# yflyl613/Tiny-NewsRec

Measured on AMD Instinct MI355X. Metric: training impressions/sec, higher is better.
Workload: dtype fp16; 1 GPU; Tiny-NewsRec 4-layer student (train [2, 3]) + 4-teacher KD (title-emb MSE + soft-CE), fwd+bwd+AMSGrad; batch_per_gpu=32, global_batch=32, user_log_length=50, candidates=5, num_words_title=30, news_dim=256, n_news=51282, parallelism=dp1

## Files before the change

include/tnr_hip.h:

```cpp
#ifndef TNR_HIP_H
#define TNR_HIP_H
#include <stdint.h>

#ifdef __cplusplus
extern "C" {
#endif

#define TNR_OK 0
#define TNR_EINVAL (-1)
#define TNR_EUNSUPPORTED (-2)
#define TNR_ELAUNCH (-3)

#define TNR_BF16 0
#define TNR_F16 1
#define TNR_F32 2

#define TNR_EPI_BIAS 1
#define TNR_EPI_GELU 2
#define TNR_EPI_TANH 4
#define TNR_EPI_RES 8
#define TNR_EPI_MULDGELU 16
#define TNR_EPI_OUTF32 32
#define TNR_EPI_AUXOUT 64
#define TNR_EPI_COLSUM 128
// ... 175 lines not shown
                         int64_t M, int64_t N, int64_t K, const float* bias, const void* res, int64_t ldres,
                         void* aux, int64_t ldaux, int flags, float* colsum_part, const tnr_dropout_t* drop,
                         const tnr_dropout_t* drop_tail, int64_t split_row, void* stream);
int tnr_ln_bwd_do_split(const void* dy, const void* x, const float* stats, const float* gamma, void* dx,
                        float* dgamma, float* dbeta, float* dxsum, float* part, int64_t M, int H, void* dxm,
                        const tnr_dropout_t* drop, const tnr_dropout_t* drop_tail, int64_t split_row, void* stream);
int tnr_attn_l32_fwd_do(const void* qkv, const float* mask_add, const float* rel, void* ctx, int64_t n_seq, int L, int A,
                        const tnr_dropout_t* drop, void* stream);
int tnr_attn_l32_bwd_do(const void* qkv, const float* mask_add, const float* rel, const void* dctx, void* dqkv,
                        float* bias_part, int64_t n_seq, int L, int A, const tnr_dropout_t* drop, void* stream);
int tnr_attn_long_fwd_do(const void* qkv, const float* mask_add, const float* rel, void* ctx, float* lse, int64_t n_seq,
                         int L, int A, const tnr_dropout_t* drop, void* stream);
int tnr_attn_long_bwd_do(const void* qkv, const float* mask_add, const float* rel, const void* ctx, const void* dctx,
                         const float* lse, float* delta, void* dqkv, int64_t n_seq, int L, int A,
                         const tnr_dropout_t* drop, void* stream);
int tnr_dropout_mask(const tnr_dropout_t* drop, int64_t rows, int64_t cols, float* out, void* stream);
int tnr_dropout_mask_probs(const tnr_dropout_t* drop, int64_t pairs, int L, int by_columns, float* out, void* stream);
int tnr_dropout_mask_split(const tnr_dropout_t* drop, const tnr_dropout_t* drop_tail, int64_t split_row, int64_t rows, int64_t cols,
                           float* out, void* stream);


int tnr_amsgrad_step(float* p, const float* g, float* m, float* v, float* vmax, int64_t n, int step,
                     float lr, float beta1, float beta2, float eps, float grad_scale, void* stream);

int tnr_grad_nonfinite(const float* g, int64_t n, unsigned* guard, unsigned stamp, void* stream);
int tnr_grad_nonfinite_scan(const float* g, int64_t n, unsigned* guard, unsigned stamp, void* stream);
int tnr_grad_nonfinite_commit(unsigned* guard, unsigned stamp, void* stream);
int tnr_amsgrad_step_guarded(float* p, const float* g, float* m, float* v, float* vmax, int64_t n, int step,
                             float lr, float beta1, float beta2, float eps, float grad_scale, const unsigned* guard,
                             unsigned stamp, unsigned known_skips, void* stream);

int tnr_refresh_shadows(const int64_t* desc, int n_desc, int64_t total_tiles, const int64_t* tile_start,
                        void* stream);

int tnr_cast_f32_to_bf16(const float* src, void* dst, int64_t n, void* stream);
int tnr_cast_bf16_to_f32(const void* src, float* dst, int64_t n, void* stream);

int tnr_embed_ln_fwd_f16(const int64_t* tok, int64_t n_seq, int L, int H, const float* word, const float* pos,
                     const float* type0, const float* gamma, const float* beta, float eps,
                     void* out, float* mask_add, void* stream);
int tnr_embed_ln_fwd_indexed_f16(const int32_t* news_combined, const int32_t* nidx, int64_t n_seq, int L, int H,
                             const float* word, const float* pos, const float* type0, const float* gamma,
                             const float* beta, float eps, void* out, float* mask_add, void* stream);
int tnr_gemm_nt_f16(const void* A, int64_t lda, const void* B, int64_t ldb, void* C, int64_t ldc,
                int64_t M, int64_t N, int64_t K, const float* bias, const void* res, int64_t ldres,
                void* aux, int64_t ldaux, int flags, void* stream);
int tnr_gemm_nt_ex_f16(const void* A, int64_t lda, const void* B, int64_t ldb, void* C, int64_t ldc,
                   int64_t M, int64_t N, int64_t K, const float* bias, const void* res, int64_t ldres,
                   void* aux, int64_t ldaux, int flags, float* colsum_part, void* stream);
int64_t tnr_gemm_colsum_rows_f16(int64_t M);
int tnr_gemm_nt_route_f16(int64_t M, int64_t N, int64_t K, int flags);
int tnr_gemm_tn_wgrad_f16(const void* dY, int64_t lddy, const void* X, int64_t ldx, float* dW, int64_t lddw,
                      int64_t M, int64_t N, int64_t K, float* ws, int splits, int accumulate, void* stream);
int tnr_gemm_tn_wgrad_ex_f16(const void* dY, int64_t lddy, const void* X, int64_t ldx, float* dW, int64_t lddw,
                         int64_t M, int64_t N, int64_t K, float* ws, int splits, int accumulate, float out_scale,
                         void* stream);
int64_t tnr_gemm_tn_ws_elems_f16(int64_t N, int64_t K, int splits);
int tnr_gemm_tn_wgrad_group_f16(const tnr_wgrad_problem_t* problems, int n, void* stream);
int tnr_ln_fwd_f16(const void* x, const float* gamma, const float* beta, float eps, void* y, float* stats,
               int64_t M, int H, void* stream);
int tnr_ln_bwd_f16(const void* dy, const void* x, const float* stats, const float* gamma, void* dx,
               float* dgamma, float* dbeta, float* dxsum, float* part, int64_t M, int H, void* stream);
int tnr_pool_fwd_f16(const void* y, float* nv, int64_t n_seq, int L, int H, int mean, void* stream);
int tnr_pool_bwd_f16(const float* dnv, void* dy, int64_t n_seq, int L, int H, int mean, void* stream);
int tnr_attn_long_fwd_f16(const void* qkv, const float* mask_add, const float* rel, void* ctx, float* lse,
                          int64_t n_seq, int L, int A, void* stream);
int tnr_attn_long_bwd_f16(const void* qkv, const float* mask_add, const float* rel, const void* ctx, const void* dctx,
                          const float* lse, float* delta, void* dqkv, int64_t n_seq, int L, int A, void* stream);
int tnr_attn_l32_fwd_f16(const void* qkv, const float* mask_add, const float* rel, void* ctx,
                     int64_t n_seq, int L, int A, void* stream);
int tnr_attn_l32_bwd_f16(const void* qkv, const float* mask_add, const float* rel, const void* dctx,
                     void* dqkv, float* bias_part, int64_t n_seq, int L, int A, void* stream);
int tnr_colsum_f16(const void* X, int64_t ldx, int dtype, int64_t M, int64_t N, float* out, float* part,
               int accumulate, void* stream);
int tnr_colsum_batched_f16(const void* X, int64_t ldx, int64_t sX, int dtype, int64_t M, int64_t N, int batch,
                       float* out, float* part, int accumulate, void* stream);
int tnr_attpool_fwd_f16(const void* y, const float* e, int64_t lde, const float* w2, const float* b2, int Q,
                    float* nv, float* alpha, float* den, int64_t n_seq, int L, int H, void* stream);
int tnr_attpool_bwd_f16(const void* y, const float* e, int64_t lde, const float* w2, int Q, const float* dnv,
                    const float* alpha, const float* den, void* dy_direct, void* dpre, int64_t lddpre,
                    float* dw2_part, float* db2_part, float* db1_part, int64_t n_seq, int L, int H, void* stream);
int64_t tnr_attpool_long_ws_elems_f16(int64_t n_seq, int L, int H, int Q, int64_t lddpre);
int tnr_attpool_fwd_long_f16(const void* y, const float* e, int64_t lde, const float* w2, const float* b2, int Q,
                         float* nv, float* alpha, float* den, float* ws, int64_t n_seq, int L, int H, void* stream);
int tnr_attpool_bwd_long_f16(const void* y, const float* e, int64_t lde, const float* w2, int Q, const float* dnv,
                         const float* alpha, void* dy_direct, void* dpre, int64_t lddpre, float* dw2_part,
                         float* db2_part, float* db1_part, float* ws, int64_t n_seq, int L, int H, void* stream);
int tnr_refresh_shadows_f16(const int64_t* desc, int n_desc, int64_t total_tiles, const int64_t* tile_start,
                        void* stream);
int tnr_cast_f32_to_bf16_f16(const float* src, void* dst, int64_t n, void* stream);
int tnr_cast_bf16_to_f32_f16(const void* src, float* dst, int64_t n, void* stream);

int tnr_embed_ln_fwd_do_f16(const int64_t* tok, int64_t n_seq, int L, int H, const float* word, const float* pos,
                        const float* type0, const float* gamma, const float* beta, float eps, void* out, float* mask_add,
                        const tnr_dropout_t* drop, const int32_t* pos_ids, void* stream);
int tnr_embed_ln_fwd_indexed_do_f16(const int32_t* news_combined, const int32_t* nidx, int64_t n_seq, int L, int H,
                                const float* word, const float* pos, const float* type0, const float* gamma,
                                const float* beta, float eps, void* out, float* mask_add, const tnr_dropout_t* drop,
                                const int32_t* pos_ids, void* stream);
int tnr_gemm_nt_do_f16(const void* A, int64_t lda, const void* B, int64_t ldb, void* C, int64_t ldc,
                   int64_t M, int64_t N, int64_t K, const float* bias, const void* res, int64_t ldres,
                   void* aux, int64_t ldaux, int flags, float* colsum_part, const tnr_dropout_t* drop, void* stream);
int tnr_ln_bwd_do_f16(const void* dy, const void* x, const float* stats, const float* gamma, void* dx,
                  float* dgamma, float* dbeta, float* dxsum, float* part, int64_t M, int H, void* dxm,
                  const tnr_dropout_t* drop, void* stream);
int tnr_gemm_nt_do_split_f16(const void* A, int64_t lda, const void* B, int64_t ldb, void* C, int64_t ldc,
                             int64_t M, int64_t N, int64_t K, const float* bias, const void* res, int64_t ldres,
                             void* aux, int64_t ldaux, int flags, float* colsum_part, const tnr_dropout_t* drop,
                             const tnr_dropout_t* drop_tail, int64_t split_row, void* stream);
int tnr_ln_bwd_do_split_f16(const void* dy, const void* x, const float* stats, const float* gamma, void* dx,
                            float* dgamma, float* dbeta, float* dxsum, float* part, int64_t M, int H, void* dxm,
                            const tnr_dropout_t* drop, const tnr_dropout_t* drop_tail, int64_t split_row, void* stream);
int tnr_attn_l32_fwd_do_f16(const void* qkv, const float* mask_add, const float* rel, void* ctx, int64_t n_seq, int L, int A,
                        const tnr_dropout_t* drop, void* stream);
int tnr_attn_l32_bwd_do_f16(const void* qkv, const float* mask_add, const float* rel, const void* dctx, void* dqkv,
                        float* bias_part, int64_t n_seq, int L, int A, const tnr_dropout_t* drop, void* stream);
int tnr_attn_long_fwd_do_f16(const void* qkv, const float* mask_add, const float* rel, void* ctx, float* lse, int64_t n_seq,
                         int L, int A, const tnr_dropout_t* drop, void* stream);
int tnr_attn_long_bwd_do_f16(const void* qkv, const float* mask_add, const float* rel, const void* ctx, const void* dctx,
                         const float* lse, float* delta, void* dqkv, int64_t n_seq, int L, int A,
                         const tnr_dropout_t* drop, void* stream);

// ... 14 lines not shown
```

tiny-newsrec_amd/csrc/optim.hip:

```cpp
#include <algorithm>

#include "common.h"

namespace {

typedef __attribute__((ext_vector_type(4))) unsigned u32x4_t;

struct AdamFactors { float lr_c1[3], inv_sqrt_c2[3]; unsigned known_skips; };
template <bool AMS>
__global__ __launch_bounds__(256) void amsgrad_kernel(float* __restrict__ p, const float* __restrict__ g,
                                                      float* __restrict__ m, float* __restrict__ v,
                                                      float* __restrict__ vmax, int64_t n, AdamFactors f,
                                                      float b1, float b2, float eps, float gscale,
                                                      const unsigned* __restrict__ guard, unsigned stamp) {
    float lr_c1 = f.lr_c1[0], inv_sqrt_c2 = f.inv_sqrt_c2[0];
    if (guard) {
        if (guard[0] == stamp) return;
        const unsigned k = guard[1] - f.known_skips;
        if (k == 1) { lr_c1 = f.lr_c1[1]; inv_sqrt_c2 = f.inv_sqrt_c2[1]; }
        else if (k >= 2) { lr_c1 = f.lr_c1[2]; inv_sqrt_c2 = f.inv_sqrt_c2[2]; }
    }
    int64_t i = ((int64_t)blockIdx.x * blockDim.x + threadIdx.x) * 4;
    if (i >= n) return;
    if (i + 4 <= n) {
// ... 56 lines not shown
                                                      const int64_t* __restrict__ tile_start) {
    __shared__ float t[32][33];
    int64_t tile = blockIdx.x;
    int di = 0;
    while (di + 1 < n_desc && tile >= tile_start[di + 1]) ++di;
    const int64_t* d = desc + (int64_t)di * 8;
    const float* src = (const float*)d[0];
    const int64_t rows = d[1], cols = d[2];
    bf16* dst = (bf16*)d[3];
    const int64_t ld = d[4];
    bf16* dstT = (bf16*)d[5];
    const int64_t ldT = d[6];
    const int64_t local = tile - tile_start[di];
    const int64_t tcols = (cols + 31) / 32;
    const int64_t r0 = (local / tcols) * 32, c0 = (local % tcols) * 32;
    const int tx = threadIdx.x & 31, ty = threadIdx.x >> 5;
#pragma unroll
    for (int k = 0; k < 4; ++k) {
        int64_t r = r0 + ty + 8 * k, c = c0 + tx;
        float v = (r < rows && c < cols) ? src[r * cols + c] : 0.f;
        t[ty + 8 * k][tx] = v;
        if (dst && r < rows && c < cols) dst[r * ld + c] = (bf16)v;
    }
    __syncthreads();
    if (dstT) {
#pragma unroll
        for (int k = 0; k < 4; ++k) {
            int64_t c = c0 + ty + 8 * k, r = r0 + tx;
            if (r < rows && c < cols) dstT[c * ldT + r] = (bf16)t[tx][ty + 8 * k];
        }
    }
}

}

#ifndef TNR_BUILD_F16
extern "C" int tnr_amsgrad_step_guarded(float* p, const float* g, float* m, float* v, float* vmax, int64_t n, int step, float lr,
                                        float beta1, float beta2, float eps, float grad_scale, const unsigned* guard,
                                        unsigned stamp, unsigned known_skips, void* stream);
extern "C" int tnr_amsgrad_step(float* p, const float* g, float* m, float* v, float* vmax, int64_t n, int step, float lr,
                                float beta1, float beta2, float eps, float grad_scale, void* stream) {
    return tnr_amsgrad_step_guarded(p, g, m, v, vmax, n, step, lr, beta1, beta2, eps, grad_scale, nullptr, 0u, 0u, stream);
}

extern "C" int tnr_grad_nonfinite_scan(const float* g, int64_t n, unsigned* guard, unsigned stamp, void* stream) {
    TNR_CHECK_ARG(g && guard && n >= 1 && stamp >= 1 && ((uintptr_t)g % 16) == 0, "tnr_grad_nonfinite_scan: bad argument");
    const unsigned grid = (unsigned)std::min<int64_t>((n + 4095) / 4096, 2048);
    hipLaunchKernelGGL(grad_nonfinite_kernel, dim3(grid), dim3(256), 0, (hipStream_t)stream, g, n, guard, stamp);
    TNR_CHECK_LAUNCH("tnr_grad_nonfinite_scan");
    return TNR_OK;
}

extern "C" int tnr_grad_nonfinite_commit(unsigned* guard, unsigned stamp, void* stream) {
    TNR_CHECK_ARG(guard && stamp >= 1, "tnr_grad_nonfinite_commit: bad argument");
    hipLaunchKernelGGL(grad_nonfinite_count_kernel, dim3(1), dim3(1), 0, (hipStream_t)stream, guard, stamp);
    TNR_CHECK_LAUNCH("tnr_grad_nonfinite_commit");
    return TNR_OK;
}

extern "C" int tnr_grad_nonfinite(const float* g, int64_t n, unsigned* guard, unsigned stamp, void* stream) {
    TNR_CHECK_ARG(g && guard && n >= 1 && stamp >= 1 && ((uintptr_t)g % 16) == 0, "tnr_grad_nonfinite: bad argument");
    const unsigned grid = (unsigned)std::min<int64_t>((n + 4095) / 4096, 2048);
    hipLaunchKernelGGL(grad_nonfinite_kernel, dim3(grid), dim3(256), 0, (hipStream_t)stream, g, n, guard, stamp);
    hipLaunchKernelGGL(grad_nonfinite_count_kernel, dim3(1), dim3(1), 0, (hipStream_t)stream, guard, stamp);
    TNR_CHECK_LAUNCH("tnr_grad_nonfinite");
    return TNR_OK;
}

extern "C" int tnr_amsgrad_step_guarded(float* p, const float* g, float* m, float* v, float* vmax, int64_t n, int step, float lr,
                                        float beta1, float beta2, float eps, float grad_scale, const unsigned* guard,
                                        unsigned stamp, unsigned known_skips, void* stream) {
    TNR_CHECK_ARG(p && g && m && v && n >= 1 && step >= 1, "tnr_amsgrad_step: bad argument");
    TNR_CHECK_ARG(((uintptr_t)p % 16) == 0 && ((uintptr_t)g % 16) == 0 && ((uintptr_t)m % 16) == 0 &&
                      ((uintptr_t)v % 16) == 0 && ((uintptr_t)vmax % 16) == 0, "tnr_amsgrad_step: 16-byte alignment");
    AdamFactors f;
    for (int k = 0; k < 3; ++k) {
        const int t = step - k >= 1 ? step - k : 1;
        const double c1 = 1.0 - pow((double)beta1, t), c2 = 1.0 - pow((double)beta2, t);
        f.lr_c1[k] = (float)((double)lr / c1);
        f.inv_sqrt_c2[k] = (float)(1.0 / sqrt(c2));
    }
    f.known_skips = known_skips;
    int64_t nthr = (n + 3) / 4;
    if (vmax)
        hipLaunchKernelGGL(amsgrad_kernel<true>, dim3((unsigned)((nthr + 255) / 256)), dim3(256), 0, (hipStream_t)stream, p, g, m,
                           v, vmax, n, f, beta1, beta2, eps, grad_scale, guard, stamp);
    else
        hipLaunchKernelGGL(amsgrad_kernel<false>, dim3((unsigned)((nthr + 255) / 256)), dim3(256), 0, (hipStream_t)stream, p, g, m,
                           v, vmax, n, f, beta1, beta2, eps, grad_scale, guard, stamp);
    TNR_CHECK_LAUNCH("tnr_amsgrad_step");
    return TNR_OK;
}

#endif

extern "C" int TNR_NAME(tnr_refresh_shadows)(const int64_t* desc, int n_desc, int64_t total_tiles, const int64_t* tile_start,
                                   void* stream) {
    TNR_CHECK_ARG(desc && tile_start && n_desc >= 1 && total_tiles >= 1, "tnr_refresh_shadows: bad argument");
    hipLaunchKernelGGL(refresh_kernel, dim3((unsigned)total_tiles), dim3(256), 0, (hipStream_t)stream, desc, n_desc,
                       tile_start);
    TNR_CHECK_LAUNCH("tnr_refresh_shadows");
    return TNR_OK;
}
```

tiny-newsrec_amd/engine.py:

```python
import logging
import math
import struct

import torch

import tnr_hip as T

PFX = "student.news_encoder."
BERT = PFX + "bert_model.bert."
QPAD = 256
AP_LONG = 64


def _rup(x, m):
    return (x + m - 1) // m * m


class EngineConfig:
    def __init__(self, n_layers=4, trainable_layers=(2, 3), hidden=768, heads=12, inter=3072, news_dim=256,
                 news_query=200, user_query=200, num_teachers=4, user_log_length=50, npratio=4, num_words=30,
                 user_log_mask=False, temperature=1.0, coef=0.2, vocab=30522, max_pos=512, type_vocab=2,
                 ln_eps=1e-12, stage1=False, pooling="att", nrms_heads=0, pos_pad_id=None):
        self.stage1 = stage1
        self.pos_pad_id = pos_pad_id
# ... 114 lines not shown
        if self.table is None:
            sb = 0 if scale == 1.0 else struct.unpack("<I", struct.pack("<f", scale))[0]
            self.jobs.append((part.data_ptr(), rows, stride, n, out.data_ptr(), int(accumulate) | (sb << 32)))

    def flush(self):
        if not self.jobs:
            return
        if self.table is None:
            l1, l2 = [], []
            for part, rows, stride, n, out, acc in self.jobs:
                chunks = max(1, min(rows // 32, 16))
                per = (rows + chunks - 1) // chunks
                chunks = (rows + per - 1) // per
                for c0 in range(0, n, 64):
                    nc = min(64, n - c0)
                    if chunks > 1:
                        for ch in range(chunks):
                            r0 = ch * per
                            src = part + 4 * (r0 * stride + c0)
                            l1.append((src, min(per, rows - r0), stride, nc, src, 0))
                        l2.append((part + 4 * c0, chunks, per * stride, nc, out + 4 * c0, acc))
                    else:
                        l2.append((part + 4 * c0, rows, stride, nc, out + 4 * c0, acc))
            mk = lambda rows_: (torch.tensor(rows_, dtype=torch.int64, device=self.dev), len(rows_)) if rows_ else None
            self.table = (mk(l1), mk(l2))
        for t in self.table:
            if t is not None:
                T.call("tnr_reduce_multi", t[0], t[1])


LOSS_SCALE = 1024.0


class LossScaler:

    def __init__(self, dev, enabled, growth_interval=2000, max_mult=64.0, min_mult=2.0 ** -20):
        self.enabled = bool(enabled) and torch.device(dev).type == "cuda"
        self.mult, self.stamp, self.clean, self.skipped, self.run_of_skips = 1.0, 0, 0, 0, 0
        self.growth_interval, self.max_mult, self.min_mult = growth_interval, max_mult, min_mult
        self.guard = torch.zeros(4, dtype=torch.int32, device=dev) if self.enabled else None
        self.pending = []
        self._ring = torch.zeros(8, dtype=torch.int32).pin_memory() if self.enabled else None

    def poll(self, eng, lag=2):
        while self.pending and self.pending[0][0] <= self.stamp - lag + 1:
            stamp, host, ev, used = self.pending.pop(0)
            ev.synchronize()
            if int(host[0]) == stamp:
                self.skipped += 1
                self.clean = 0
                self.run_of_skips += 1
                self.mult = max(min(self.mult, used * 0.5), self.min_mult)
                eng.step_count = max(eng.step_count - 1, 0)
                if self.run_of_skips == 16:
                    logging.warning("16 optimiser steps in a row skipped for inf / nan gradients although the loss scale went down "
                                    "to %g: the fp16 FORWARD overflows (or the data holds inf / nan) - use --dtype bf16", eng.gscale)
            else:
                self.run_of_skips = 0
                self.clean += 1
                if self.clean >= self.growth_interval and self.mult < self.max_mult:
                    self.mult, self.clean = self.mult * 2.0, 0

    def record(self, used):
        host = self._ring[self.stamp % 8: self.stamp % 8 + 1]
        host.copy_(self.guard[:1], non_blocking=True)
        ev = torch.cuda.Event()
        ev.record()
        self.pending.append((self.stamp, host, ev, used))

    def drain(self, eng):
        self.poll(eng, lag=0)

    def reset(self, eng):
        self.drain(eng)
        self.mult, self.clean, self.run_of_skips = 1.0, 0, 0


class Engine:
    def __init__(self, cfg, device="cuda:0", max_batch=32, dtype="fp16", share=None, extra_rows=0, extra_seqs=0):
        T.lib()
        assert dtype in ("bf16", "fp16")
        self.f16 = dtype == "fp16"
        self.dtype = dtype
        self.tdt = torch.float16 if self.f16 else torch.bfloat16
        self._gbase = LOSS_SCALE if self.f16 else 1.0
        self.cfg, self.dev = cfg, torch.device(device)
        self.scaler = share.scaler if share is not None else LossScaler(self.dev, self.f16)
        self.step_count = 0
        self._n_alloc = 0
        if share is None:
            self._build_params()
            self._build_shadows()
        else:
            for k in ("shapes", "slot", "n_train", "n_frozen", "flat", "flat_g", "adam_m", "adam_v", "adam_vmax", "params",
                      "grads", "lo", "sh", "sh_a1", "sh_a1T", "b_a1", "desc_all", "desc_train"):
                setattr(self, k, getattr(share, k))
        self.max_batch = max_batch
        self.extra_rows, self.extra_seqs = int(extra_rows), int(extra_seqs)
        self.drop = None
        self.drop_calls = 0
        self._alloc_workspace(max_batch)
        self.comm = None

    @property
    def gscale(self):
        return self._gbase * self.scaler.mult

    @property
    def ginv(self):
        return 1.0 / self.gscale

    def _groups(self):
        cfg = self.cfg
        T_ = cfg.T
        tstack = lambda suffix: ["teachers.%d.%s" % (i, suffix) for i in range(T_)]
        groups = []
        if T_ and cfg.nrms_heads and not cfg.stage1:
            groups.append((["teachers.%d.%s" % (i, n) for i in range(T_) for n in NRMS_W], None))
            groups.append((["teachers.%d.%s" % (i, n) for i in range(T_) for n in NRMS_B], None))
        if T_ and not cfg.stage1:
            for suffix in ("attn.att_fc1.weight", "attn.att_fc1.bias", "attn.att_fc2.weight", "pad_doc", "attn.att_fc2.bias"):
                groups.append((tstack(suffix), None))
        for k in ("word_embeddings.weight", "position_embeddings.weight", "token_type_embeddings.weight",
                  "LayerNorm.weight", "LayerNorm.bias"):
            groups.append(([BERT + "embeddings." + k], None))
        for l in range(cfg.n_layers):
            n = layer_param_order(l)
            groups.append((n[0:3], None))
# ... 113 lines not shown
        cfg, dev, bf = self.cfg, self.dev, self.tdt
        H, I = cfg.H, cfg.I
        lo = min(cfg.trainable_layers) if cfg.trainable_layers else cfg.n_layers
        self.lo = lo
        self.sh = []
        for l in range(cfg.n_layers):
            d = dict(qkv=torch.zeros((3 * H, H), device=dev, dtype=bf), o=torch.zeros((H, H), device=dev, dtype=bf),
                     w1=torch.zeros((I, H), device=dev, dtype=bf), w2=torch.zeros((H, I), device=dev, dtype=bf))
            if l >= lo:
                d.update(qkvT=torch.zeros((H, 3 * H), device=dev, dtype=bf), oT=torch.zeros((H, H), device=dev, dtype=bf),
                         w1T=torch.zeros((H, I), device=dev, dtype=bf), w2T=torch.zeros((I, H), device=dev, dtype=bf))
            self.sh.append(d)
        self.sh_a1 = torch.zeros((QPAD, H), device=dev, dtype=bf)
        self.sh_a1T = torch.zeros((H, QPAD), device=dev, dtype=bf)
        self.b_a1 = self._view(PFX + "attn.att_fc1.bias", QPAD, (QPAD,)) if cfg.pooling == "att" else None

        def table(layers, with_heads):
            rows = []
            for l in layers:
                d, names = self.sh[l], layer_param_order(l)
                for i in range(3):
                    rows.append((self.p(names[i]), H, H, d["qkv"][i * H:], H, d["qkvT"][:, i * H:] if "qkvT" in d else None, 3 * H))
                rows.append((self.p(names[6]), H, H, d["o"], H, d.get("oT"), H))
                rows.append((self.p(names[10]), I, H, d["w1"], H, d.get("w1T"), I))
                rows.append((self.p(names[12]), H, I, d["w2"], I, d.get("w2T"), H))
            if with_heads and cfg.pooling == "att":
                rows.append((self.p(PFX + "attn.att_fc1.weight"), cfg.Qn, H, self.sh_a1, H, self.sh_a1T, QPAD))
            desc, start, tot = [], [0], 0
            for src, r, c, dst, ld, dstT, ldT in rows:
                desc.append([src.data_ptr(), r, c, dst.data_ptr(), ld, dstT.data_ptr() if dstT is not None else 0, ldT, 0])
                tot += ((r + 31) // 32) * ((c + 31) // 32)
                start.append(tot)
            return (torch.tensor(desc, dtype=torch.int64, device=dev), len(desc), tot,
                    torch.tensor(start, dtype=torch.int64, device=dev))

        self.desc_all = table(range(cfg.n_layers), True)
        self.desc_train = table(cfg.trainable_layers, True)

    def refresh_shadows(self, all_layers=False):
        d = self.desc_all if all_layers else self.desc_train
        self._c("tnr_refresh_shadows", d[0], d[1], d[2], d[3])
        if all_layers:
            self.fcache = None
            self.refresh_rel()

    def refresh_rel(self):
        T.call("tnr_relpos_table", self.p(BERT + "rel_pos_bias.weight"), self.cfg.A, self.cfg.L, self.rel)
        self._rel_stale = False

    def _alloc_workspace(self, B):
        cfg, dev, bf = self.cfg, self.dev, self.tdt
        H, I, D, L = cfg.H, cfg.I, cfg.D, cfg.L
        N = B * (cfg.U + cfg.C)
        Mp = _rup(N * L + self.extra_rows, 128)
        self.B_alloc, self.N_alloc, self.Mp = B, N, Mp
        Nx = N + self.extra_seqs
        if self.f16:
            k = 0
            while (32 << k) < B and k < 5:
                k += 1
            self._gbase = LOSS_SCALE * (1 << k)
        z = lambda *s, dt=bf: torch.zeros(s, device=dev, dtype=dt)
        f = lambda *s: torch.zeros(s, device=dev, dtype=torch.float32)
        Lr = _rup(L, 32)
        self.Lr = Lr
        self.tok = torch.zeros((N, 2 * L), device=dev, dtype=torch.int64)
        self.nidx_buf = torch.zeros(N, device=dev, dtype=torch.int32)
        self.mask_add = f(N, Lr)
        self.rel = f(cfg.A, Lr, Lr)
        self.lse = f(N, cfg.A, Lr) if L > 32 else None
# ... 638 lines not shown
    def grad(self, name):
        return self.grads[name]

    def bucket_ranges(self):
        out = [(self.off(PFX + ("attn.att_fc1.weight" if self.cfg.pooling == "att" else "dense.weight")), self.n_train)]
        for l in sorted(self.cfg.trainable_layers, reverse=True):
            names = layer_param_order(l)
            a0, f0 = self.off(names[0]), self.off(names[10])
            e = self.off(names[-1]) + self.slot[names[-1]][2]
            out.append((f0, _rup(e, 64)))
            out.append((a0, f0))
        return out

    def step(self, lr, grad_scale=1.0, beta1=0.9, beta2=0.999, eps=1e-8, lr_bert=None, amsgrad=True, lr_news_head=None, sync=None):
        sc = self.scaler
        guard, stamp = None, 0
        if sc.enabled:
            used = sc.mult
            sc.poll(self)
            sc.stamp += 1
            guard, stamp = sc.guard, sc.stamp
        self.step_count += 1
        head0 = self.off(PFX + ("attn.att_fc1.weight" if self.cfg.pooling == "att" else "dense.weight"))
        e = self.off(PFX + "dense.bias") + self.slot[PFX + "dense.bias"][2]
        rest0 = min(_rup(e, 64), self.n_train)
        lb = lr if lr_bert is None else lr_bert
        lh = lr if lr_news_head is None else lr_news_head
        ranges = []
        for lo_, hi_, rate in ((0, head0, lb), (head0, rest0, lh), (rest0, self.n_train, lr)):
            if ranges and ranges[-1][2] == rate and ranges[-1][1] == lo_:
                ranges[-1] = (ranges[-1][0], hi_, rate)
            elif hi_ > lo_:
                ranges.append((lo_, hi_, rate))
        def launch(lo_, hi_, rate):
            if hi_ > lo_:
                args = (self.flat[True][lo_:hi_], self.flat_g[lo_:hi_], self.adam_m[lo_:hi_], self.adam_v[lo_:hi_],
                        self.adam_vmax[lo_:hi_] if amsgrad else None, hi_ - lo_, self.step_count, rate, beta1, beta2, eps, grad_scale)
                if guard is None:
                    T.call("tnr_amsgrad_step", *args)
                else:
                    T.call("tnr_amsgrad_step_guarded", *args, guard, stamp, sc.skipped)

        if guard is not None:
            if sync is not None and sync.pending:
                for b, (s_, e_) in enumerate(sync.ranges):
                    sync.wait_bucket(b)
                    T.call("tnr_grad_nonfinite_scan", self.flat_g[s_:e_], e_ - s_, guard, stamp)
                T.call("tnr_grad_nonfinite_commit", guard, stamp)
            else:
                if sync is not None:
                    sync.wait()
                T.call("tnr_grad_nonfinite", self.flat_g, self.n_train, guard, stamp)
            for lo_, hi_, rate in ranges:
                launch(lo_, hi_, rate)
            sc.record(used)
        elif sync is not None and sync.pending:
            done = []
            for b, (s_, e_) in enumerate(sync.ranges):
                sync.wait_bucket(b)
                for lo_, hi_, rate in ranges:
                    launch(max(lo_, s_), min(hi_, e_), rate)
                done.append((s_, e_))
            pos = 0
            for s_, e_ in sorted(done) + [(self.n_train, self.n_train)]:
                for lo_, hi_, rate in ranges:
                    launch(max(lo_, pos), min(hi_, s_), rate)
                pos = max(pos, e_)
        else:
            if sync is not None:
                sync.wait()
            for lo_, hi_, rate in ranges:
                launch(lo_, hi_, rate)
        self.refresh_shadows(all_layers=False)
```

tiny-newsrec_amd/tnr_hip.py:

```python
import ctypes
import os

import torch

_HERE = os.path.dirname(os.path.abspath(__file__))
LIB_PATH = os.path.join(_HERE, "csrc", "libtnr_hip.so")

BF16, F16, F32 = 0, 1, 2
ROUTE_128, ROUTE_256x128, ROUTE_256, ROUTE_224 = 128, 2128, 256, 224
EPI_BIAS, EPI_GELU, EPI_TANH, EPI_RES, EPI_MULDGELU, EPI_OUTF32, EPI_AUXOUT, EPI_COLSUM = 1, 2, 4, 8, 16, 32, 64, 128

_c = ctypes
_P, _I, _L, _F = _c.c_void_p, _c.c_int, _c.c_int64, _c.c_float

DROP_EMB, DROP_PROB, DROP_ATTN_OUT, DROP_FFN_OUT = 0, 1, 2, 3


class Dropout(_c.Structure):
    _fields_ = [("seed", _c.c_uint64), ("site", _c.c_uint32), ("call", _c.c_uint32), ("p", _c.c_double)]

    @classmethod
    def site_of(cls, p, seed, kind, layer, call):
        if p is None or p <= 0.0:
            return None
# ... 93 lines not shown
    "tnr_attpool_fwd": [_P, _P, _L, _P, _P, _I, _P, _P, _P, _L, _I, _I, _P],
    "tnr_attpool_bwd": [_P, _P, _L, _P, _I, _P, _P, _P, _P, _P, _L, _P, _P, _P, _L, _I, _I, _P],
    "tnr_attpool_fwd_long": [_P, _P, _L, _P, _P, _I, _P, _P, _P, _P, _L, _I, _I, _P],
    "tnr_attpool_bwd_long": [_P, _P, _L, _P, _I, _P, _P, _P, _P, _L, _P, _P, _P, _P, _L, _I, _I, _P],
    "tnr_sgemm": [_P, _L, _L, _L, _P, _P, _L, _L, _L, _P, _L, _L, _P, _L, _L, _L, _L, _I, _F, _F, _I, _P, _P],
    "tnr_sgemm_group": [_c.POINTER(SgemmProblem), _I, _P],
    "tnr_gemm_tn_wgrad_group": [_c.POINTER(WgradProblem), _I, _P],
    "tnr_concat_i32": [_P, _L, _P, _L, _P, _P],
    "tnr_gather_rows": [_P, _L, _P, _L, _I, _I, _P, _L, _L, _P],
    "tnr_segment_sum_rows": [_P, _P, _P, _L, _I, _P, _P],
    "tnr_user_score_fwd": [_P, _L, _P, _P, _P, _P, _P, _P, _P, _P, _I, _P, _P, _P, _L, _P, _P, _P, _P, _I, _I, _I, _I, _I, _I, _P],
    "tnr_user_bwd_pre": [_P, _P, _P, _P, _P, _I, _P, _P, _P, _P, _P, _P, _I, _I, _I, _I, _P],
    "tnr_user_bwd_post": [_P, _P, _P, _P, _P, _I, _P, _P, _I, _I, _I, _I, _P],
    "tnr_user_bwd_part_stride": [_I, _I],
    "tnr_user_blend_fwd": [_P, _L, _P, _P, _P, _I, _P, _I, _I, _I, _I, _P],
    "tnr_user_blend_bwd": [_P, _P, _P, _I, _P, _P, _L, _I, _I, _I, _P],
    "tnr_nrms_attn_fwd": [_P, _P, _I, _P, _L, _I, _I, _I, _I, _P],
    "tnr_nrms_attn_bwd": [_P, _P, _I, _P, _P, _I, _I, _I, _P],
    "tnr_score_bwd": [_P, _P, _P, _P, _P, _P, _I, _I, _I, _P],
    "tnr_kd_score_loss": [_P, _P, _P, _F, _F, _P, _P, _P, _I, _I, _I, _P],
    "tnr_kd_embed_loss": [_P, _P, _P, _P, _P, _P, _P, _I, _I, _I, _I, _I, _P],
    "tnr_reduce_rows": [_P, _L, _L, _L, _P, _I, _P],
    "tnr_reduce_multi": [_P, _I, _P],
    "tnr_dropout_mask": [_D, _L, _L, _P, _P],
    "tnr_dropout_mask_probs": [_D, _L, _I, _I, _P, _P],
    "tnr_dropout_mask_split": [_D, _D, _L, _L, _L, _P, _P],
    "tnr_scale_inplace": [_P, _L, _F, _P],
    "tnr_amsgrad_step": [_P, _P, _P, _P, _P, _L, _I, _F, _F, _F, _F, _F, _P],
    "tnr_amsgrad_step_guarded": [_P, _P, _P, _P, _P, _L, _I, _F, _F, _F, _F, _F, _P, _c.c_uint, _c.c_uint, _P],
    "tnr_grad_nonfinite": [_P, _L, _P, _c.c_uint, _P],
    "tnr_grad_nonfinite_scan": [_P, _L, _P, _c.c_uint, _P],
    "tnr_grad_nonfinite_commit": [_P, _c.c_uint, _P],
    "tnr_refresh_shadows": [_P, _I, _L, _P, _P],
    "tnr_cast_f32_to_bf16": [_P, _P, _L, _P],
    "tnr_cast_bf16_to_f32": [_P, _P, _L, _P],
}
TYPED = ["tnr_embed_ln_fwd", "tnr_embed_ln_fwd_indexed", "tnr_gemm_nt", "tnr_gemm_nt_ex", "tnr_gemm_colsum_rows", "tnr_gemm_nt_route",
         "tnr_gemm_tn_wgrad", "tnr_gemm_tn_wgrad_ex", "tnr_gemm_tn_wgrad_group", "tnr_gemm_tn_ws_elems", "tnr_ln_fwd", "tnr_ln_bwd", "tnr_attn_l32_fwd", "tnr_attn_l32_bwd", "tnr_attn_long_fwd", "tnr_attn_long_bwd",
         "tnr_colsum", "tnr_colsum_batched", "tnr_attpool_fwd", "tnr_attpool_bwd", "tnr_attpool_fwd_long", "tnr_attpool_bwd_long", "tnr_attpool_long_ws_elems", "tnr_refresh_shadows",
         "tnr_cast_f32_to_bf16", "tnr_cast_bf16_to_f32", "tnr_pool_fwd", "tnr_pool_bwd"]
for _n in ("tnr_embed_ln_fwd", "tnr_embed_ln_fwd_indexed", "tnr_attn_l32_fwd", "tnr_attn_l32_bwd", "tnr_attn_long_fwd", "tnr_attn_long_bwd"):
    _SIG[_n + "_do"] = _SIG[_n][:-1] + [_D] + ([_P] if "embed" in _n else []) + [_P]
    TYPED.append(_n + "_do")
_SIG["tnr_gemm_nt_do"] = _SIG["tnr_gemm_nt_ex"][:-1] + [_D, _P]
_SIG["tnr_ln_bwd_do"] = _SIG["tnr_ln_bwd"][:-1] + [_P, _D, _P]
_SIG["tnr_gemm_nt_do_split"] = _SIG["tnr_gemm_nt_do"][:-1] + [_D, _L, _P]
_SIG["tnr_ln_bwd_do_split"] = _SIG["tnr_ln_bwd_do"][:-1] + [_D, _L, _P]
TYPED += ["tnr_gemm_nt_do", "tnr_ln_bwd_do", "tnr_gemm_nt_do_split", "tnr_ln_bwd_do_split"]
for _n in TYPED:
    _SIG[_n + "_f16"] = _SIG[_n]
_RET = {"tnr_attpool_long_ws_elems": _L, "tnr_attpool_long_ws_elems_f16": _L, "tnr_gemm_tn_ws_elems": _L, "tnr_gemm_tn_ws_elems_f16": _L, "tnr_gemm_colsum_rows_f16": _L, "tnr_gemm_colsum_rows": _L, "tnr_ln_bwd_part_elems": _L, "tnr_ln_bwd_blocks": _L, "tnr_colsum_part_elems": _L,
        "tnr_user_bwd_part_stride": _L}
EXPORTS = sorted(_SIG) + ["tnr_last_error"]

_lib = None


class TnrError(RuntimeError):
    pass


def lib():
    global _lib
    if _lib is None:
        if not os.path.exists(LIB_PATH):
            raise TnrError("libtnr_hip.so not built: run `make -C tiny-newsrec_amd/csrc` (or __graft_entry__.build())")
        L = ctypes.CDLL(LIB_PATH)
        for name, args in _SIG.items():
            fn = getattr(L, name)
            fn.argtypes = args
            fn.restype = _RET.get(name, _I)
        L.tnr_last_error.restype = ctypes.c_char_p
# ... 75 lines not shown
```

Before: 4242 impressions/s.

## Fuse AMSGrad step with bf16 shadow weight refresh in one kernel

Adds a kernel that runs the AMSGrad update per 64x64 tile of each trainable weight matrix and writes the bf16 shadow copy and its transpose straight from registers through shared memory. Parameter ranges outside any matrix are updated as flat 4096-element chunks. This removes the separate shadow-refresh pass that re-read the updated fp32 parameters, and saves a launch. The cost is a descriptor table built and cached per optimizer range, plus more complex tail handling.

```diff
diff --git a/include/tnr_hip.h b/include/tnr_hip.h
--- a/include/tnr_hip.h
+++ b/include/tnr_hip.h
@@ -231,6 +231,11 @@
 
 int tnr_refresh_shadows(const int64_t* desc, int n_desc, int64_t total_tiles, const int64_t* tile_start,
                         void* stream);
+
+int tnr_amsgrad_step_refresh(float* p, const float* g, float* m, float* v, float* vmax, int64_t n, int step,
+                             float lr, float beta1, float beta2, float eps, float grad_scale, const unsigned* guard,
+                             unsigned stamp, unsigned known_skips, const int64_t* desc, int n_desc, int64_t total_units,
+                             const int64_t* unit_start, void* stream);
 
 int tnr_cast_f32_to_bf16(const float* src, void* dst, int64_t n, void* stream);
 int tnr_cast_bf16_to_f32(const void* src, float* dst, int64_t n, void* stream);
@@ -287,6 +292,10 @@
                          float* db2_part, float* db1_part, float* ws, int64_t n_seq, int L, int H, void* stream);
 int tnr_refresh_shadows_f16(const int64_t* desc, int n_desc, int64_t total_tiles, const int64_t* tile_start,
                         void* stream);
+int tnr_amsgrad_step_refresh_f16(float* p, const float* g, float* m, float* v, float* vmax, int64_t n, int step,
+                             float lr, float beta1, float beta2, float eps, float grad_scale, const unsigned* guard,
+                             unsigned stamp, unsigned known_skips, const int64_t* desc, int n_desc, int64_t total_units,
+                             const int64_t* unit_start, void* stream);
 int tnr_cast_f32_to_bf16_f16(const float* src, void* dst, int64_t n, void* stream);
 int tnr_cast_bf16_to_f32_f16(const void* src, float* dst, int64_t n, void* stream);
 
diff --git a/tiny-newsrec_amd/csrc/optim.hip b/tiny-newsrec_amd/csrc/optim.hip
--- a/tiny-newsrec_amd/csrc/optim.hip
+++ b/tiny-newsrec_amd/csrc/optim.hip
@@ -112,6 +112,198 @@
     }
 }
 
+AdamFactors adam_factors(int step, float lr, float beta1, float beta2, unsigned known_skips) {
+    AdamFactors f;
+    for (int k = 0; k < 3; ++k) {
+        const int t = step - k >= 1 ? step - k : 1;
+        const double c1 = 1.0 - pow((double)beta1, t), c2 = 1.0 - pow((double)beta2, t);
+        f.lr_c1[k] = (float)((double)lr / c1);
+        f.inv_sqrt_c2[k] = (float)(1.0 / sqrt(c2));
+    }
+    f.known_skips = known_skips;
+    return f;
+}
+
+struct AdamArgs { float lr_c1, inv_sqrt_c2, b1, b2, eps, gscale; };
+template <bool AMS>
+__device__ __forceinline__ void adam_update4(f32x4 graw, f32x4& mv, f32x4& vv, f32x4& vm, f32x4& pv, const AdamArgs& a) {
+    const float b1 = a.b1, b2 = a.b2, eps = a.eps, lr_c1 = a.lr_c1, inv_sqrt_c2 = a.inv_sqrt_c2;
+    f32x4 gv = graw * a.gscale;
+    mv = mv * b1 + (1.f - b1) * gv;
+    vv = vv * b2 + (1.f - b2) * gv * gv;
+    if (!AMS) vm = vv;
+#pragma unroll
+    for (int r = 0; r < 4; ++r) {
+        if (AMS) vm[r] = fmaxf(vm[r], vv[r]);
+        pv[r] -= lr_c1 * (mv[r] / (sqrtf(vm[r]) * inv_sqrt_c2 + eps));
+    }
+}
+template <bool AMS>
+__device__ __forceinline__ float adam_update1(float* p, const float* g, float* m, float* v, float* vmax, int64_t i, const AdamArgs& a) {
+    const float b1 = a.b1, b2 = a.b2, eps = a.eps, lr_c1 = a.lr_c1, inv_sqrt_c2 = a.inv_sqrt_c2;
+    float gv = g[i] * a.gscale;
+    float mv = m[i] * b1 + (1.f - b1) * gv;
+    float vv = v[i] * b2 + (1.f - b2) * gv * gv;
+    float vm = AMS ? fmaxf(vmax[i], vv) : vv;
+    m[i] = mv; v[i] = vv;
+    if (AMS) vmax[i] = vm;
+    p[i] -= lr_c1 * (mv / (sqrtf(vm) * inv_sqrt_c2 + eps));
+    return p[i];
+}
+
+template <bool AMS>
+__device__ __forceinline__ void adam_update_some(float* p, const float* g, float* m, float* v, float* vmax, int64_t i, int cnt,
+                                                 int64_t tail, const AdamArgs& a, float out[4]) {
+    f32x4 G = {0.f, 0.f, 0.f, 0.f}, M = G, V = G, X = G, P = G;
+#pragma unroll
+    for (int j = 0; j < 4; ++j)
+        if (j < cnt && i + j < tail) {
+            G[j] = g[i + j]; M[j] = m[i + j]; V[j] = v[i + j]; P[j] = p[i + j];
+            if (AMS) X[j] = vmax[i + j];
+        }
+    adam_update4<AMS>(G, M, V, X, P, a);
+#pragma unroll
+    for (int j = 0; j < 4; ++j)
+        if (j < cnt) {
+            if (i + j < tail) {
+                m[i + j] = M[j]; v[i + j] = V[j]; p[i + j] = P[j];
+                if (AMS) vmax[i + j] = X[j];
+                out[j] = P[j];
+            } else {
+                out[j] = adam_update1<AMS>(p, g, m, v, vmax, i + j, a);
+            }
+        }
+}
+
+constexpr int FT = 64;
+constexpr int FCHUNK = 4096;
+template <bool AMS>
+__global__ __launch_bounds__(256) void amsgrad_refresh_kernel(float* __restrict__ p, const float* __restrict__ g,
+                                                              float* __restrict__ m, float* __restrict__ v,
+                                                              float* __restrict__ vmax, int64_t n, AdamFactors f,
+                                                              float b1, float b2, float eps, float gscale,
+                                                              const unsigned* __restrict__ guard, unsigned stamp,
+                                                              const int64_t* __restrict__ desc, int n_desc,
+                                                              const int64_t* __restrict__ unit_start) {
+    __shared__ __attribute__((aligned(16))) bf16 tT[FT][FT + 4];
+    AdamArgs a = {f.lr_c1[0], f.inv_sqrt_c2[0], b1, b2, eps, gscale};
+    if (guard) {
+        if (guard[0] == stamp) return;
+        const unsigned k = guard[1] - f.known_skips;
+        if (k == 1) { a.lr_c1 = f.lr_c1[1]; a.inv_sqrt_c2 = f.inv_sqrt_c2[1]; }
+        else if (k >= 2) { a.lr_c1 = f.lr_c1[2]; a.inv_sqrt_c2 = f.inv_sqrt_c2[2]; }
+    }
+    const int64_t unit = blockIdx.x;
+    int di = 0, hi = n_desc - 1;
+    while (di < hi) {
+        const int mid = (di + hi + 1) >> 1;
+        if (unit_start[mid] <= unit) di = mid; else hi = mid - 1;
+    }
+    const int64_t* d = desc + (int64_t)di * 8;
+    const int64_t rows = d[1], cols = d[2];
+    const int64_t off = (const float*)d[0] - p;
+    if (rows < 1 || cols < 1 || off < 0 || off + rows * cols > n) return;
+    bf16* dst = (bf16*)d[3];
+    const int64_t ld = d[4];
+    bf16* dstT = (bf16*)d[5];
+    const int64_t ldT = d[6];
+    const int64_t local = unit - unit_start[di];
+    const int tid = threadIdx.x;
+    p += off; g += off; m += off; v += off;
+    if (AMS) vmax += off;
+    const int64_t tail = (n & ~(int64_t)3) - off;
+    const bool vec_in = (off & 3) == 0;
+
+    if (!dst && !dstT) {
+        const int64_t len = rows * cols, e0 = local * FCHUNK;
+        f32x4 G[4], M[4], V[4], X[4], P[4];
+        bool full[4];
+#pragma unroll
+        for (int u = 0; u < 4; ++u) {
+            const int64_t i = e0 + tid * 4 + u * 1024;
+            full[u] = vec_in && i + 4 <= len;
+            if (full[u]) {
+                G[u] = *(const f32x4*)(g + i); M[u] = *(const f32x4*)(m + i); V[u] = *(const f32x4*)(v + i);
+                if (AMS) X[u] = *(const f32x4*)(vmax + i);
+                P[u] = *(const f32x4*)(p + i);
+            }
+        }
+#pragma unroll
+        for (int u = 0; u < 4; ++u) {
+            const int64_t i = e0 + tid * 4 + u * 1024;
+            if (full[u]) {
+                adam_update4<AMS>(G[u], M[u], V[u], X[u], P[u], a);
+                *(f32x4*)(m + i) = M[u]; *(f32x4*)(v + i) = V[u];
+                if (AMS) *(f32x4*)(vmax + i) = X[u];
+                *(f32x4*)(p + i) = P[u];
+            } else {
+                float out[4];
+                if (i < len) adam_update_some<AMS>(p, g, m, v, vmax, i, (int)(len - i < 4 ? len - i : 4), tail, a, out);
+            }
+        }
+        return;
+    }
+
+    const int64_t tcols = (cols + FT - 1) / FT;
+    const int64_t r0 = (local / tcols) * FT, c0 = (local % tcols) * FT;
+    if (r0 >= rows) return;
+    const int lx = tid & 15, ly = tid >> 4;
+    const bool vec_row = vec_in && (cols & 3) == 0;
+    const bool vec_dst = dst && (ld & 3) == 0 && ((uintptr_t)dst & 7) == 0;
+    const int64_t c = c0 + 4 * lx;
+    f32x4 G[4], M[4], V[4], X[4], P[4];
+    bool full[4];
+#pragma unroll
+    for (int k = 0; k < 4; ++k) {
+        const int64_t r = r0 + ly + 16 * k, i = r * cols + c;
+        full[k] = vec_row && r < rows && c + 4 <= cols;
+        if (full[k]) {
+            G[k] = *(const f32x4*)(g + i); M[k] = *(const f32x4*)(m + i); V[k] = *(const f32x4*)(v + i);
+            if (AMS) X[k] = *(const f32x4*)(vmax + i);
+            P[k] = *(const f32x4*)(p + i);
+        }
+    }
+#pragma unroll
+    for (int k = 0; k < 4; ++k) {
+        const int rl = ly + 16 * k;
+        const int64_t r = r0 + rl, i = r * cols + c;
+        if (full[k]) {
+            adam_update4<AMS>(G[k], M[k], V[k], X[k], P[k], a);
+            *(f32x4*)(m + i) = M[k]; *(f32x4*)(v + i) = V[k];
+            if (AMS) *(f32x4*)(vmax + i) = X[k];
+            *(f32x4*)(p + i) = P[k];
+            bf16x4 h;
+#pragma unroll
+            for (int j = 0; j < 4; ++j) { h[j] = (bf16)P[k][j]; tT[4 * lx + j][rl] = h[j]; }
+            if (vec_dst) *(bf16x4*)(dst + r * ld + c) = h;
+            else if (dst)
+                for (int j = 0; j < 4; ++j) dst[r * ld + c + j] = h[j];
+        } else if (r < rows) {
+            float out[4];
+            const int cnt = (int)(cols - c < 4 ? cols - c : 4);
+            if (cnt > 0) adam_update_some<AMS>(p, g, m, v, vmax, i, cnt, tail, a, out);
+            for (int j = 0; j < cnt; ++j) {
+                const bf16 h = (bf16)out[j];
+                tT[4 * lx + j][rl] = h;
+                if (dst) dst[r * ld + c + j] = h;
+            }
+        }
+    }
+    if (!dstT) return;
+    __syncthreads();
+    const bool vec_T = (ldT & 3) == 0 && ((uintptr_t)dstT & 7) == 0;
+    const int64_t r = r0 + 4 * lx;
+#pragma unroll
+    for (int k = 0; k < 4; ++k) {
+        const int cl = ly + 16 * k;
+        const int64_t cc = c0 + cl;
+        if (cc >= cols) continue;
+        if (vec_T && r + 4 <= rows) *(bf16x4*)(dstT + cc * ldT + r) = *(const bf16x4*)&tT[cl][4 * lx];
+        else
+            for (int j = 0; j < 4 && r + j < rows; ++j) dstT[cc * ldT + r + j] = tT[cl][4 * lx + j];
+    }
+}
+
 }
 
 #ifndef TNR_BUILD_F16
@@ -153,14 +345,7 @@
     TNR_CHECK_ARG(p && g && m && v && n >= 1 && step >= 1, "tnr_amsgrad_step: bad argument");
     TNR_CHECK_ARG(((uintptr_t)p % 16) == 0 && ((uintptr_t)g % 16) == 0 && ((uintptr_t)m % 16) == 0 &&
                       ((uintptr_t)v % 16) == 0 && ((uintptr_t)vmax % 16) == 0, "tnr_amsgrad_step: 16-byte alignment");
-    AdamFactors f;
-    for (int k = 0; k < 3; ++k) {
-        const int t = step - k >= 1 ? step - k : 1;
-        const double c1 = 1.0 - pow((double)beta1, t), c2 = 1.0 - pow((double)beta2, t);
-        f.lr_c1[k] = (float)((double)lr / c1);
-        f.inv_sqrt_c2[k] = (float)(1.0 / sqrt(c2));
-    }
-    f.known_skips = known_skips;
+    const AdamFactors f = adam_factors(step, lr, beta1, beta2, known_skips);
     int64_t nthr = (n + 3) / 4;
     if (vmax)
         hipLaunchKernelGGL(amsgrad_kernel<true>, dim3((unsigned)((nthr + 255) / 256)), dim3(256), 0, (hipStream_t)stream, p, g, m,
@@ -182,3 +367,24 @@
     TNR_CHECK_LAUNCH("tnr_refresh_shadows");
     return TNR_OK;
 }
+
+extern "C" int TNR_NAME(tnr_amsgrad_step_refresh)(float* p, const float* g, float* m, float* v, float* vmax, int64_t n, int step,
+                                                  float lr, float beta1, float beta2, float eps, float grad_scale,
+                                                  const unsigned* guard, unsigned stamp, unsigned known_skips,
+                                                  const int64_t* desc, int n_desc, int64_t total_units, const int64_t* unit_start,
+                                                  void* stream) {
+    TNR_CHECK_ARG(p && g && m && v && n >= 1 && step >= 1, "tnr_amsgrad_step_refresh: bad argument");
+    TNR_CHECK_ARG(((uintptr_t)p % 16) == 0 && ((uintptr_t)g % 16) == 0 && ((uintptr_t)m % 16) == 0 &&
+                      ((uintptr_t)v % 16) == 0 && ((uintptr_t)vmax % 16) == 0, "tnr_amsgrad_step_refresh: 16-byte alignment");
+    TNR_CHECK_ARG(desc && unit_start && n_desc >= 1 && total_units >= 1 && total_units <= 0x7FFFFFFF,
+                  "tnr_amsgrad_step_refresh: bad descriptor table");
+    const AdamFactors f = adam_factors(step, lr, beta1, beta2, known_skips);
+    if (vmax)
+        hipLaunchKernelGGL(amsgrad_refresh_kernel<true>, dim3((unsigned)total_units), dim3(256), 0, (hipStream_t)stream, p, g, m, v,
+                           vmax, n, f, beta1, beta2, eps, grad_scale, guard, stamp, desc, n_desc, unit_start);
+    else
+        hipLaunchKernelGGL(amsgrad_refresh_kernel<false>, dim3((unsigned)total_units), dim3(256), 0, (hipStream_t)stream, p, g, m, v,
+                           vmax, n, f, beta1, beta2, eps, grad_scale, guard, stamp, desc, n_desc, unit_start);
+    TNR_CHECK_LAUNCH("tnr_amsgrad_step_refresh");
+    return TNR_OK;
+}
diff --git a/tiny-newsrec_amd/engine.py b/tiny-newsrec_amd/engine.py
--- a/tiny-newsrec_amd/engine.py
+++ b/tiny-newsrec_amd/engine.py
@@ -170,6 +170,25 @@
 LOSS_SCALE = 1024.0
 
 
+FUSED_TILE, FUSED_CHUNK = 64, 4096
+
+
+def fused_rows(mats, lo, hi):
+    out, pos = [], lo
+    flat = lambda a, b: out.append((a, 1, b - a, None, -(-(b - a) // FUSED_CHUNK)))
+    for i, (o, r, c) in sorted(enumerate(mats), key=lambda t: t[1][0]):
+        if not lo <= o < hi:
+            continue
+        assert o >= pos and o + r * c <= hi, "weight matrix at %d (%d x %d) overlaps its neighbour or leaves [%d, %d)" % (o, r, c, lo, hi)
+        if o > pos:
+            flat(pos, o)
+        out.append((o, r, c, i, -(-r // FUSED_TILE) * -(-c // FUSED_TILE)))
+        pos = o + r * c
+    if hi > pos:
+        flat(pos, hi)
+    return out
+
+
 class LossScaler:
 
     def __init__(self, dev, enabled, growth_interval=2000, max_mult=64.0, min_mult=2.0 ** -20):
@@ -231,7 +250,7 @@
             self._build_shadows()
         else:
             for k in ("shapes", "slot", "n_train", "n_frozen", "flat", "flat_g", "adam_m", "adam_v", "adam_vmax", "params",
-                      "grads", "lo", "sh", "sh_a1", "sh_a1T", "b_a1", "desc_all", "desc_train"):
+                      "grads", "lo", "sh", "sh_a1", "sh_a1T", "b_a1", "desc_all", "desc_train", "rows_train", "_fused_tabs"):
                 setattr(self, k, getattr(share, k))
         self.max_batch = max_batch
         self.extra_rows, self.extra_seqs = int(extra_rows), int(extra_seqs)
@@ -411,10 +430,27 @@
                 tot += ((r + 31) // 32) * ((c + 31) // 32)
                 start.append(tot)
             return (torch.tensor(desc, dtype=torch.int64, device=dev), len(desc), tot,
-                    torch.tensor(start, dtype=torch.int64, device=dev))
-
-        self.desc_all = table(range(cfg.n_layers), True)
-        self.desc_train = table(cfg.trainable_layers, True)
+                    torch.tensor(start, dtype=torch.int64, device=dev), rows)
+
+        self.desc_all = table(range(cfg.n_layers), True)[:4]
+        *self.desc_train, self.rows_train = table(cfg.trainable_layers, True)
+        self._fused_tabs = {}
+
+    def _fused_table(self, lo_, hi_):
+        tab = self._fused_tabs.get((lo_, hi_))
+        if tab is None:
+            flat, rows = self.flat[True], self.rows_train
+            base, ptr = flat.data_ptr(), lambda t: t.data_ptr() if t is not None else 0
+            mats = [((src.data_ptr() - base) // 4, r, c) for src, r, c, dst, ld, dstT, ldT in rows]
+            desc, start = [], [0]
+            for o, r, c, i, units in fused_rows(mats, lo_, hi_):
+                _, _, _, dst, ld, dstT, ldT = rows[i] if i is not None else (None, 0, 0, None, 0, None, 0)
+                desc.append([base + 4 * o, r, c, ptr(dst), ld, ptr(dstT), ldT, 0])
+                start.append(start[-1] + units)
+            dev = self.dev
+            tab = self._fused_tabs[(lo_, hi_)] = (torch.tensor(desc, dtype=torch.int64, device=dev), len(desc), start[-1],
+                                                  torch.tensor(start, dtype=torch.int64, device=dev))
+        return tab
 
     def refresh_shadows(self, all_layers=False):
         d = self.desc_all if all_layers else self.desc_train
@@ -1119,11 +1155,15 @@
                 ranges[-1] = (ranges[-1][0], hi_, rate)
             elif hi_ > lo_:
                 ranges.append((lo_, hi_, rate))
+        fused = getattr(self, "fused_optim", True) and not (sync is not None and sync.pending)
         def launch(lo_, hi_, rate):
             if hi_ > lo_:
                 args = (self.flat[True][lo_:hi_], self.flat_g[lo_:hi_], self.adam_m[lo_:hi_], self.adam_v[lo_:hi_],
                         self.adam_vmax[lo_:hi_] if amsgrad else None, hi_ - lo_, self.step_count, rate, beta1, beta2, eps, grad_scale)
-                if guard is None:
+                if fused:
+                    self._c("tnr_amsgrad_step_refresh", *args, guard, stamp, sc.skipped if guard is not None else 0,
+                            *self._fused_table(lo_, hi_))
+                elif guard is None:
                     T.call("tnr_amsgrad_step", *args)
                 else:
                     T.call("tnr_amsgrad_step_guarded", *args, guard, stamp, sc.skipped)
@@ -1158,4 +1198,5 @@
                 sync.wait()
             for lo_, hi_, rate in ranges:
                 launch(lo_, hi_, rate)
-        self.refresh_shadows(all_layers=False)
+        if not fused:
+            self.refresh_shadows(all_layers=False)
diff --git a/tiny-newsrec_amd/tnr_hip.py b/tiny-newsrec_amd/tnr_hip.py
--- a/tiny-newsrec_amd/tnr_hip.py
+++ b/tiny-newsrec_amd/tnr_hip.py
@@ -149,12 +149,13 @@
     "tnr_grad_nonfinite_scan": [_P, _L, _P, _c.c_uint, _P],
     "tnr_grad_nonfinite_commit": [_P, _c.c_uint, _P],
     "tnr_refresh_shadows": [_P, _I, _L, _P, _P],
+    "tnr_amsgrad_step_refresh": [_P, _P, _P, _P, _P, _L, _I, _F, _F, _F, _F, _F, _P, _c.c_uint, _c.c_uint, _P, _I, _L, _P, _P],
     "tnr_cast_f32_to_bf16": [_P, _P, _L, _P],
     "tnr_cast_bf16_to_f32": [_P, _P, _L, _P],
 }
 TYPED = ["tnr_embed_ln_fwd", "tnr_embed_ln_fwd_indexed", "tnr_gemm_nt", "tnr_gemm_nt_ex", "tnr_gemm_colsum_rows", "tnr_gemm_nt_route",
          "tnr_gemm_tn_wgrad", "tnr_gemm_tn_wgrad_ex", "tnr_gemm_tn_wgrad_group", "tnr_gemm_tn_ws_elems", "tnr_ln_fwd", "tnr_ln_bwd", "tnr_attn_l32_fwd", "tnr_attn_l32_bwd", "tnr_attn_long_fwd", "tnr_attn_long_bwd",
-         "tnr_colsum", "tnr_colsum_batched", "tnr_attpool_fwd", "tnr_attpool_bwd", "tnr_attpool_fwd_long", "tnr_attpool_bwd_long", "tnr_attpool_long_ws_elems", "tnr_refresh_shadows",
+         "tnr_colsum", "tnr_colsum_batched", "tnr_attpool_fwd", "tnr_attpool_bwd", "tnr_attpool_fwd_long", "tnr_attpool_bwd_long", "tnr_attpool_long_ws_elems", "tnr_refresh_shadows", "tnr_amsgrad_step_refresh",
          "tnr_cast_f32_to_bf16", "tnr_cast_bf16_to_f32", "tnr_pool_fwd", "tnr_pool_bwd"]
 for _n in ("tnr_embed_ln_fwd", "tnr_embed_ln_fwd_indexed", "tnr_attn_l32_fwd", "tnr_attn_l32_bwd", "tnr_attn_long_fwd", "tnr_attn_long_bwd"):
     _SIG[_n + "_do"] = _SIG[_n][:-1] + [_D] + ([_P] if "embed" in _n else []) + [_P]
```

Result: no change. 4250 impressions/s (median of 6 runs) (+0.2%).
